# kpmrozowski/wut-cuda-orb-slam3

Hardware: NVIDIA B200
Metric: orb_extract_frames_per_s_752x480_1000kp (higher is better)
Workload: dtype u8

## Files before the change

### wut_cuda_orb_slam3_b200/csrc/api.cu

```cuda
#include <algorithm>
#include <atomic>
#include <climits>
#include <cfloat>
#include <cmath>
#include <cstdarg>
#include <cstdio>
#include <cstdlib>
#include <cstring>
#include <mutex>
#include <string>
#include <unordered_map>
#include <vector>

#include "orbx_internal.cuh"
#include "introsort_replay.h"
#include "synth.h"

namespace orbx {

static thread_local std::string t_err;
static std::atomic<long long> g_launches{0};

void count_launch(int n) { g_launches.fetch_add(n, std::memory_order_relaxed); }

int fail(int code, const char* fmt, ...)
{
    char buf[512];
    va_list ap;
    va_start(ap, fmt);
    vsnprintf(buf, sizeof buf, fmt, ap);
    va_end(ap);
    t_err = buf;
    return code;
}

#define CU(call)                                                                                         \
// ... 566 lines not shown
{
    if (!ex->profiling) return ORBX_OK;
    if (ex->ev_used == ex->ev_pool.size()) {
        cudaEvent_t e;
        CU(cudaEventCreate(&e));
        ex->ev_pool.push_back(e);
    }
    CU(cudaEventRecord(ex->ev_pool[ex->ev_used++], st));
    return ORBX_OK;
}

static int run_chunk(orbx_extractor* ex, Slot& s, const uint8_t* d_images, size_t frame_stride, size_t pitch, int frames,
                     int lap0, int lap1, orbx_keypoint* d_kps, uint8_t* d_desc, int capacity, int* d_n, int* d_nm,
                     cudaStream_t st)
{
    const FrameGeom& fg = ex->fg;
    int rc;
    ex->mirror_valid = false;
    if ((rc = prof_mark(ex, st))) return rc;
    CU(launch_pyramid(fg, s.ws, d_images, frame_stride, pitch, frames, st));
    if ((rc = prof_mark(ex, st))) return rc;
    static const char* fork_env = getenv("ORBX_BATCH_FORK");
    const bool fork = (fork_env ? atoi(fork_env) != 0 : true) && !ex->profiling && frames >= 8;
    if (fork) {
        if (!ex->side[0]) CU(cudaStreamCreateWithFlags(&ex->side[0], cudaStreamNonBlocking));
        if (!ex->ev_lvl[0]) CU(cudaEventCreateWithFlags(&ex->ev_lvl[0], cudaEventDisableTiming));
        if (!ex->ev_side[0]) CU(cudaEventCreateWithFlags(&ex->ev_side[0], cudaEventDisableTiming));
        CU(cudaEventRecord(ex->ev_lvl[0], st));
        CU(cudaStreamWaitEvent(ex->side[0], ex->ev_lvl[0], 0));
        CU(launch_fast(fg, s.ws, frames, st));
        CU(launch_blur(fg, s.ws, frames, ex->side[0]));
        CU(cudaEventRecord(ex->ev_side[0], ex->side[0]));
        CU(launch_octree(fg, s.ws, frames, st));
        CU(cudaStreamWaitEvent(st, ex->ev_side[0], 0));
    } else {
        CU(launch_fast(fg, s.ws, frames, st));
        if ((rc = prof_mark(ex, st))) return rc;
        CU(launch_blur(fg, s.ws, frames, st));
        if ((rc = prof_mark(ex, st))) return rc;
        CU(launch_octree(fg, s.ws, frames, st));
    }
    if ((rc = prof_mark(ex, st))) return rc;
    bool fused = false;
    CU(launch_orient_describe(fg, s.ws, frames, st, lap0, lap1, d_kps, d_desc, capacity, d_n, d_nm, &fused));
    if ((rc = prof_mark(ex, st))) return rc;
    if (!fused) CU(launch_pack(fg, s.ws, frames, lap0, lap1, d_kps, d_desc, capacity, d_n, d_nm, st));
    if ((rc = prof_mark(ex, st))) return rc;
    return ORBX_OK;
}

static int run_single_forked(orbx_extractor* ex, Slot& s, const uint8_t* d_image, size_t pitch, int lap0, int lap1,
                             orbx_keypoint* d_kps, uint8_t* d_desc, int capacity, int* d_n, int* d_nm, cudaStream_t st)
{
    const FrameGeom& fg = ex->fg;
    for (int l = 0; l < fg.nlevels; ++l) {
        if (!ex->side[l]) CU(cudaStreamCreateWithFlags(&ex->side[l], cudaStreamNonBlocking));
        if (!ex->ev_lvl[l]) CU(cudaEventCreateWithFlags(&ex->ev_lvl[l], cudaEventDisableTiming));
        if (!ex->ev_side[l]) CU(cudaEventCreateWithFlags(&ex->ev_side[l], cudaEventDisableTiming));
    }
    for (int l = 0; l < fg.nlevels; ++l) {
        CU(launch_pyramid(fg, s.ws, d_image, pitch * fg.rows, pitch, 1, st, l, l + 1));
        CU(cudaEventRecord(ex->ev_lvl[l], st));
        if (ex->mirror) {
            const LevelGeom& g = fg.L[l];
            const size_t bw = (size_t)g.w + 2 * kEdge;
            CU(cudaStreamWaitEvent(ex->mirror_stream, ex->ev_lvl[l], 0));
            CU(cudaMemcpy2DAsync(ex->h_mirror + ex->mirror_off[l], bw, s.ws.pyr + g.pyr_off + (kXPad - kEdge), g.pitch, bw, (size_t)g.rows_alloc,
// ... 1040 lines not shown
```

### wut_cuda_orb_slam3_b200/csrc/kernels_describe.cu

```cuda
#include <float.h>

#include <algorithm>
#include <cstdlib>
#include <mutex>

#include "orbx_internal.cuh"

namespace orbx {

namespace {

__constant__ int c_umax[16] = {15, 15, 15, 15, 14, 14, 14, 13, 13, 12, 11, 10, 9, 8, 6, 3};

__device__ float4 d_pattern_f[8][32];
__device__ uint4 d_mom_mask[16][2];

constexpr int BT_W = 128, BT_H = 32;
constexpr int BIN_P = 160;
constexpr int BIN_R = BT_H + 6;

__device__ __forceinline__ float fast_atan2_dev(float y, float x)
{
    const float scale = (float)(180.0 / 3.14159265358979323846);
    const float p1 = 0.9997878412794807f * scale, p3 = -0.3258083974640975f * scale;
    const float p5 = 0.1555786518463281f * scale, p7 = -0.04432655554792128f * scale;
    const float ax = fabsf(x), ay = fabsf(y);
    float a, c, c2;
    if (ax >= ay) {
        c = __fdiv_rn(ay, __fadd_rn(ax, (float)DBL_EPSILON));
        c2 = __fmul_rn(c, c);
        a = __fmul_rn(__fadd_rn(__fmul_rn(__fadd_rn(__fmul_rn(__fadd_rn(__fmul_rn(p7, c2), p5), c2), p3), c2), p1), c);
    } else {
        c = __fdiv_rn(ax, __fadd_rn(ay, (float)DBL_EPSILON));
        c2 = __fmul_rn(c, c);
        a = __fsub_rn(90.f, __fmul_rn(__fadd_rn(__fmul_rn(__fadd_rn(__fmul_rn(__fadd_rn(__fmul_rn(p7, c2), p5), c2), p3), c2), p1), c));
    }
    if (x < 0) a = __fsub_rn(180.f, a);
    if (y < 0) a = __fsub_rn(360.f, a);
    return a;
}

}

__global__ void __launch_bounds__(256) blur_kernel(const __grid_constant__ FrameGeom fg, Workspace ws)
{
    __shared__ __align__(128) uint8_t in[BIN_R * BIN_P];
    __shared__ __align__(16) uint32_t hb[BIN_R * BT_W];
    __shared__ __align__(16) uint8_t outt[BT_H * BT_W];
    const int tid = threadIdx.x;
    const int frame = blockIdx.y;
    int t = blockIdx.x, level = 0, tx_n = 0;
#pragma unroll 1
    for (int l = 0; l < fg.nlevels; ++l) {
        tx_n = (fg.L[l].w + BT_W - 1) / BT_W;
        const int nt = tx_n * ((fg.L[l].h + BT_H - 1) / BT_H);
        if (t < nt) { level = l; break; }
        t -= nt;
    }
    const LevelGeom& g = fg.L[level];
    const int tyi = t / tx_n;
    const int ty0 = tyi * BT_H, tx0 = (t - tyi * tx_n) * BT_W;
    const uint8_t* base = ws.pyr + g.pyr_off + (size_t)frame * g.pyr_frame_stride;
    const int brow0 = ty0 - 3 + kEdge, bcol0 = tx0 - 16 + kXPad;
// ... 200 lines not shown
            for (int r = 0; r < rows; r += 7) {
#pragma unroll
                for (int kk = 0; kk < 7; ++kk) {
                    if (r + kk < rows) {
                        hrow(r + kk + 6, W[(kk + 6) % 7]);
                        uint32_t o = 0;
#pragma unroll
                        for (int j = 0; j < 4; ++j) {
                            const uint32_t sum = 18u * (W[kk % 7][j] + W[(kk + 6) % 7][j]) + 34u * (W[(kk + 1) % 7][j] + W[(kk + 5) % 7][j]) +
                                                 48u * (W[(kk + 2) % 7][j] + W[(kk + 4) % 7][j]) + 56u * W[(kk + 3) % 7][j];
                            o |= ((sum + 32768u) >> 16) << (8 * j);
                        }
                        *reinterpret_cast<uint32_t*>(out) = o;
                        out += bpitch;
                    }
                }
            }
        }
        __syncwarp();
        if (lane == 0 && item + kBpStages * nw < total_items) issue(item + kBpStages * nw, sgi);
    }
}

struct FusedPack {
    int mode;
    orbx_keypoint* kps; uint8_t* desc; int capacity; int* n_out; int* n_mono;
};

constexpr int kOdStage = kDescBoxW * kDescBoxH;
#ifndef ORBX_OD_MINB
#define ORBX_OD_MINB 5
#endif

template <bool STAGED>
__global__ void __launch_bounds__(256, STAGED ? ORBX_OD_MINB : 1) orient_describe_kernel(const __grid_constant__ FrameGeom fg, Workspace ws, FusedPack fp)
{
    extern __shared__ __align__(128) uint8_t od_smem[];
    __shared__ __align__(8) uint64_t od_bar[8];
    const int lane = threadIdx.x & 31;
    const int slot = blockIdx.x * 8 + (threadIdx.x >> 5);
    const int frame = blockIdx.y;
    if (slot >= fg.kp_slots) return;
    static_assert((kMaxLevels & (kMaxLevels - 1)) == 0, "binary search over a power of two");
    int level = 0;
#pragma unroll
    for (int step = kMaxLevels / 2; step >= 1; step >>= 1)
        if (slot >= fg.L[level + step].kp_base) level += step;
    const LevelGeom& g = fg.L[level];
    const int i = slot - g.kp_base;
    int n_level, t_out = 0, nkp = 0;
    if (fp.mode) {
        const int c = lane < fg.nlevels ? ws.lvl_n[(size_t)frame * fg.nlevels + lane] : 0;
        int incl = c;
#pragma unroll
        for (int d = 1; d < 32; d <<= 1) {
            const int t = __shfl_up_sync(0xffffffffu, incl, d);
            if (lane >= d) incl += t;
        }
        n_level = __shfl_sync(0xffffffffu, c, level);
        t_out = __shfl_sync(0xffffffffu, incl - c, level) + i;
        nkp = __shfl_sync(0xffffffffu, incl, 31);
        if (slot == 0 && lane == 0) {
            fp.n_out[frame] = nkp;
            fp.n_mono[frame] = nkp > fp.capacity ? -1 : (fp.mode == 1 ? nkp : 0);
        }
    } else {
        n_level = ws.lvl_n[(size_t)frame * fg.nlevels + level];
    }
    if (i >= n_level) return;
    const uint32_t key = ws.lvl_kp[(size_t)frame * fg.kp_slots + slot];
    const int x = (int)(key & 0xfff) + kWinBorder, y = (int)((key >> 12) & 0xfff) + kWinBorder;

    constexpr bool staged = STAGED;
    const int warp = threadIdx.x >> 5;
    const int x0 = (x - 19) & ~15;
    const uint32_t stage_s = (uint32_t)__cvta_generic_to_shared(od_smem) + (uint32_t)warp * kOdStage;
    if (staged) {
        if (lane == 0) {
            mbar_init(&od_bar[warp], 1);
            mbar_expect_tx(&od_bar[warp], kDescBoxW * kDescBoxH);
            tma_load_3d(od_smem + warp * kOdStage, ws.tmap_desc + level, &od_bar[warp], x0, y - 20, frame);
        }
        __syncwarp();
    }

    int m10 = 0, m01 = 0;
    {
        const int v = lane - kHalfPatch;
        if (lane < 31) {
            const uint8_t* rowp = level_interior((const uint8_t*)ws.pyr, g, frame) + (ptrdiff_t)(y + v) * g.pitch + (x - kHalfPatch);
            const int mis16 = (int)((uintptr_t)rowp & 15);
            const int mis = mis16 & 3;
            const uint4* rq = reinterpret_cast<const uint4*>(rowp - mis16);
            const uint4 q0 = __ldg(rq), q1 = __ldg(rq + 1), q2 = __ldg(rq + 2);
            uint32_t w[12] = {q0.x, q0.y, q0.z, q0.w, q1.x, q1.y, q1.z, q1.w, q2.x, q2.y, q2.z, q2.w};
            if (mis16 & 4) {
#pragma unroll
                for (int j = 0; j < 11; ++j) w[j] = w[j + 1];
            }
            if (mis16 & 8) {
#pragma unroll
                for (int j = 0; j < 10; ++j) w[j] = w[j + 2];
            }
            const int av = v < 0 ? -v : v;
            const uint4 ma = d_mom_mask[av][0], mb = d_mom_mask[av][1];
            const uint32_t mk[8] = {ma.x, ma.y, ma.z, ma.w, mb.x, mb.y, mb.z, mb.w};
            const int sh = 8 * mis;
            int sum = 0;
#pragma unroll
            for (int j = 0; j < 8; ++j) {
                const uint32_t px = __funnelshift_r(w[j], w[j + 1], sh) & mk[j];
                const int u0 = -kHalfPatch + 4 * j;
                const uint32_t wt = (uint32_t)(u0 & 0xff) | ((uint32_t)((u0 + 1) & 0xff) << 8) | ((uint32_t)((u0 + 2) & 0xff) << 16) |
                                    ((uint32_t)((u0 + 3) & 0xff) << 24);
                asm("dp4a.u32.s32 %0, %1, %2, %0;" : "+r"(m10) : "r"(px), "r"(wt));
                sum = (int)__dp4a(px, 0x01010101u, (uint32_t)sum);
            }
            m01 = v * sum;
        }
#pragma unroll
        for (int d = 16; d >= 1; d >>= 1) {
            m10 += __shfl_xor_sync(0xffffffffu, m10, d);
            m01 += __shfl_xor_sync(0xffffffffu, m01, d);
        }
    }
    const float angle = fast_atan2_dev((float)m01, (float)m10);

    const float factorPI = (float)(3.14159265358979323846 / 180.f);
    const float arad = __fmul_rn(angle, factorPI);
    double sd, cd;
    sincos((double)arad, &sd, &cd);
    const float a = (float)cd, b = (float)sd;
    const uint8_t* center = ws.blur + g.blur_off + (size_t)frame * g.blur_frame_stride + (size_t)y * g.bpitch + x;
    const int step = g.bpitch;
    const float kMagic = 12582912.0f;
    const int kMagicBits = 0x4B400000;
    uint32_t val = 0;
    if (staged) {
        mbar_wait(&od_bar[warp], 0);
        const uint32_t cb = stage_s + 20 * kDescBoxW + (uint32_t)(x - x0);
#pragma unroll
        for (int k = 0; k < 8; ++k) {
            const float4 q = d_pattern_f[k][lane];
            const int iy0 = __float_as_int(__fadd_rn(__fadd_rn(__fmul_rn(q.x, b), __fmul_rn(q.y, a)), kMagic)) - kMagicBits;
            const int ix0 = __float_as_int(__fadd_rn(__fsub_rn(__fmul_rn(q.x, a), __fmul_rn(q.y, b)), kMagic)) - kMagicBits;
            const int iy1 = __float_as_int(__fadd_rn(__fadd_rn(__fmul_rn(q.z, b), __fmul_rn(q.w, a)), kMagic)) - kMagicBits;
            const int ix1 = __float_as_int(__fadd_rn(__fsub_rn(__fmul_rn(q.z, a), __fmul_rn(q.w, b)), kMagic)) - kMagicBits;
            uint32_t t0, t1;
            asm volatile("ld.shared.u8 %0, [%1];" : "=r"(t0) : "r"(cb + (uint32_t)(iy0 * kDescBoxW + ix0)));
            asm volatile("ld.shared.u8 %0, [%1];" : "=r"(t1) : "r"(cb + (uint32_t)(iy1 * kDescBoxW + ix1)));
            val |= (uint32_t)(t0 < t1) << k;
        }
    } else
#pragma unroll
    for (int k = 0; k < 8; ++k) {
        const float4 q = d_pattern_f[k][lane];
        const int iy0 = __float_as_int(__fadd_rn(__fadd_rn(__fmul_rn(q.x, b), __fmul_rn(q.y, a)), kMagic)) - kMagicBits;
        const int ix0 = __float_as_int(__fadd_rn(__fsub_rn(__fmul_rn(q.x, a), __fmul_rn(q.y, b)), kMagic)) - kMagicBits;
        const int iy1 = __float_as_int(__fadd_rn(__fadd_rn(__fmul_rn(q.z, b), __fmul_rn(q.w, a)), kMagic)) - kMagicBits;
        const int ix1 = __float_as_int(__fadd_rn(__fsub_rn(__fmul_rn(q.z, a), __fmul_rn(q.w, b)), kMagic)) - kMagicBits;
        const int t0 = __ldg(center + iy0 * step + ix0), t1 = __ldg(center + iy1 * step + ix1);
        val |= (uint32_t)(t0 < t1) << k;
    }
    ws.lvl_desc[((size_t)frame * fg.kp_slots + slot) * 32 + lane] = (uint8_t)val;
    if (lane == 0) ws.lvl_angle[(size_t)frame * fg.kp_slots + slot] = angle;
    if (fp.mode && nkp <= fp.capacity) {
        const int dst = fp.mode == 1 ? t_out : nkp - 1 - t_out;
        fp.desc[((size_t)frame * fp.capacity + dst) * 32 + lane] = (uint8_t)val;
        if (lane < 7) {
            float px = (float)x, py = (float)y;
            if (level != 0) { px = __fmul_rn(px, g.scale); py = __fmul_rn(py, g.scale); }
            uint32_t w;
            switch (lane) {
                case 0: w = __float_as_uint(px); break;
                case 1: w = __float_as_uint(py); break;
                case 2: w = __float_as_uint(g.kp_size); break;
                case 3: w = __float_as_uint(angle); break;
                case 4: w = __float_as_uint((float)(key >> 24)); break;
                case 5: w = (uint32_t)level; break;
                default: w = 0xffffffffu; break;
            }
            reinterpret_cast<uint32_t*>(fp.kps + (size_t)frame * fp.capacity + dst)[lane] = w;
        }
    }
}

template <int T>
__global__ void __launch_bounds__(T) pack_kernel(const __grid_constant__ FrameGeom fg, Workspace ws, int lap0, int lap1,
                                                 orbx_keypoint* __restrict__ kps, uint8_t* __restrict__ desc, int capacity,
                                                 int* __restrict__ n_out, int* __restrict__ n_mono)
{
    __shared__ int lvl_off[kMaxLevels + 1];
    __shared__ int warp_cnt[T / 32];
    __shared__ int carry;
    const int tid = threadIdx.x, lane = tid & 31, warp = tid >> 5;
    const int frame = blockIdx.x;
    if (warp == 0) {
        static_assert(kMaxLevels <= 32, "one lane per level");
        const int c = lane < fg.nlevels ? ws.lvl_n[(size_t)frame * fg.nlevels + lane] : 0;
        int incl = c;
#pragma unroll
        for (int d = 1; d < 32; d <<= 1) {
            const int t = __shfl_up_sync(0xffffffffu, incl, d);
            if (lane >= d) incl += t;
        }
        if (lane < fg.nlevels) lvl_off[lane] = incl - c;
        if (lane == fg.nlevels - 1) lvl_off[fg.nlevels] = incl;
// ... 99 lines not shown
    };
    static const int umax[16] = {15, 15, 15, 15, 14, 14, 14, 13, 13, 12, 11, 10, 9, 8, 6, 3};
    float4 pf[8][32];
    for (int lane = 0; lane < 32; ++lane)
        for (int k = 0; k < 8; ++k) {
            const int8_t* t = pat + 4 * (8 * lane + k);
            pf[k][lane] = make_float4((float)t[0], (float)t[1], (float)t[2], (float)t[3]);
        }
    uint32_t mask[16][8];
    for (int av = 0; av < 16; ++av)
        for (int j = 0; j < 8; ++j) {
            uint32_t m = 0;
            for (int bb = 0; bb < 4; ++bb) {
                const int u = -15 + 4 * j + bb;
                if ((u < 0 ? -u : u) <= umax[av]) m |= 0xffu << (8 * bb);
            }
            mask[av][j] = m;
        }
    cudaError_t e = cudaMemcpyToSymbol(d_pattern_f, pf, sizeof pf);
    if (e != cudaSuccess) return e;
    return cudaMemcpyToSymbol(d_mom_mask, mask, sizeof mask);
}

cudaError_t launch_orient_describe(const FrameGeom& fg, const Workspace& ws, int n_frames, cudaStream_t st, int lap0, int lap1,
                                   orbx_keypoint* d_kps, uint8_t* d_desc, int capacity, int* d_n_out, int* d_n_mono, bool* fused)
{
    FusedPack fp{};
    static const bool no_fuse = getenv("ORBX_NO_FUSED_PACK") != nullptr;
    if (d_kps && d_desc && d_n_out && d_n_mono && !no_fuse && fg.kp_slots > 0 && n_frames < 8) {
        if (lap1 < kEdge || lap0 >= fg.cols || lap0 > lap1) fp.mode = 1;
        else if (lap0 <= kEdge && lap1 >= fg.cols) fp.mode = 2;
        fp.kps = d_kps; fp.desc = d_desc; fp.capacity = capacity; fp.n_out = d_n_out; fp.n_mono = d_n_mono;
    }
    if (fused) *fused = fp.mode != 0;
    static bool filled[64] = {false};
    static std::mutex mu;
    int dev = 0;
    cudaGetDevice(&dev);
    std::lock_guard<std::mutex> lock(mu);
    if (!filled[dev & 63]) {
        cudaError_t e = fill_describe_tables();
        if (e != cudaSuccess) return e;
        filled[dev & 63] = true;
    }
    dim3 grid((fg.kp_slots + 7) / 8, n_frames);
    static const char* od_env = getenv("ORBX_DESC_STAGED");
    if (ws.tmap_desc && (od_env ? atoi(od_env) != 0 : true)) orient_describe_kernel<true><<<grid, 256, 8 * kOdStage, st>>>(fg, ws, fp);
    else orient_describe_kernel<false><<<grid, 256, 0, st>>>(fg, ws, fp);
    count_launch();
    return cudaGetLastError();
}

cudaError_t launch_pack(const FrameGeom& fg, const Workspace& ws, int n_frames, int lap0, int lap1, orbx_keypoint* d_kps,
                        uint8_t* d_desc, int capacity, int* d_n_out, int* d_n_mono, cudaStream_t st)
{
    if (n_frames >= 8) pack_kernel<256><<<n_frames, 256, 0, st>>>(fg, ws, lap0, lap1, d_kps, d_desc, capacity, d_n_out, d_n_mono);
    else pack_kernel<1024><<<n_frames, 1024, 0, st>>>(fg, ws, lap0, lap1, d_kps, d_desc, capacity, d_n_out, d_n_mono);
    count_launch();
    return cudaGetLastError();
}

}
```

### wut_cuda_orb_slam3_b200/csrc/kernels_octree.cu

```cuda
#include <stdlib.h>

#include <mutex>

#include "introsort_replay.h"
#include "orbx_internal.cuh"

namespace orbx {

namespace {

constexpr int kSortBitsMax = 12;

struct Smem {
    int* bstart;
    int* cursor;
    int* warp_tmp;
    int* sort_stk;
    uint32_t* nbeg[2];
    uint32_t* ncnt[2];
    uint32_t* nx[2];
    uint32_t* ndep[2];
    uint32_t* npre[2];
    uint32_t* cc;
    int* sa;
    int* sb;
    int* sc;
// ... 199 lines not shown
__host__ __device__ inline int octree_sort_depth(int depth, int root_bits)
{
    const int d = (kSortBitsMax - root_bits) / 2;
    return d < depth ? (d > 0 ? d : 0) : depth;
}

int octree_bins(const LevelGeom& g) { return 1 << (g.root_bits + 2 * octree_sort_depth(g.depth, g.root_bits)); }

size_t octree_smem_bytes(int M, int NB)
{
    size_t b = 0;
    b += sizeof(uint32_t) * (size_t)M * 10;
    b += sizeof(uint32_t) * (size_t)M * 4;
    b += sizeof(int) * (size_t)M * 5;
    b += 8;
    b += sizeof(unsigned long long) * (size_t)M * 2;
    const size_t cur = sizeof(int) * (size_t)NB;
    return sizeof(int) * (64 + 224) + sizeof(int) * ((size_t)NB + 2) + (b > cur ? b : cur);
}

#ifndef ORBX_OCT_THREADS_PER_SM
#define ORBX_OCT_THREADS_PER_SM 1024
#endif
template <int T>
__global__ void __launch_bounds__(T, ORBX_OCT_THREADS_PER_SM / T) octree_kernel(const __grid_constant__ FrameGeom fg, Workspace ws, int M, int NB,
                                                   int level_base, int* __restrict__ err_flag)
{
    extern __shared__ __align__(16) unsigned char smem_raw[];
    __shared__ int s_nL, s_nS, s_total;

    const int tid = threadIdx.x, lane = tid & 31, warp = tid >> 5;
    const int frame = blockIdx.x, level = level_base + blockIdx.y;
    const LevelGeom& g = fg.L[level];
    const int N = g.nfeat;
    long long* dbg = (ws.dbg && frame == 0 && level == ws.dbg_level && tid == 0) ? ws.dbg : nullptr;
    long long t_prev = dbg ? clock64() : 0;
#define OCT_MARK(slot) do { if (dbg) { const long long t_now = clock64(); dbg[slot] += t_now - t_prev; t_prev = t_now; } } while (0)
    long long t_fine = t_prev;
#define OCT_FINE(slot) do { if (dbg) { const long long t_now = clock64(); dbg[slot] += t_now - t_fine; t_fine = t_now; } } while (0)
    const int winW = g.w - 2 * kWinBorder, winH = g.h - 2 * kWinBorder;

    Smem S;
    {
        unsigned char* p = smem_raw;
        S.warp_tmp = (int*)p; p += sizeof(int) * 64;
        S.sort_stk = (int*)p; p += sizeof(int) * 224;
        S.bstart = (int*)p; p += sizeof(int) * ((size_t)NB + 2);
        S.cursor = (int*)p;
        for (int b = 0; b < 2; ++b) {
            S.nbeg[b] = (uint32_t*)p; p += 4 * (size_t)M;
            S.ncnt[b] = (uint32_t*)p; p += 4 * (size_t)M;
// ... 313 lines not shown
            const int i = i0 + u;
            if (i < nL) {
                const uint32_t beg = S.nbeg[a][i], cnt = S.ncnt[a][i];
                for (uint32_t j = lane; j < cnt; j += 32) {
                    const uint32_t pl = K[beg + j], kk = K2[beg + j];
                    const unsigned long long v = ((unsigned long long)((pl & 0xff000000u) | (0xffffffu - (pl & 0xffffffu))) << 32) | kk;
                    best[u] = v > best[u] ? v : best[u];
                }
            }
        }
#pragma unroll
        for (int u = 0; u < RU; ++u) {
#pragma unroll
            for (int d = 16; d >= 1; d >>= 1) {
                const unsigned long long o = __shfl_xor_sync(0xffffffffu, best[u], d);
                best[u] = o > best[u] ? o : best[u];
            }
            if (lane == 0 && i0 + u < nL) out_kp[i0 + u] = (uint32_t)best[u];
        }
    }
    if (tid == 0) *out_n = nL;
    OCT_MARK(6);
    if (dbg) dbg[9] = n;
#undef OCT_MARK
#undef OCT_FINE
}

cudaError_t octree_prepare()
{
    cudaError_t e = cudaFuncSetAttribute(octree_kernel<256>, cudaFuncAttributeMaxDynamicSharedMemorySize, 200 * 1024);
    if (e != cudaSuccess) return e;
    e = cudaFuncSetAttribute(octree_kernel<64>, cudaFuncAttributeMaxDynamicSharedMemorySize, 200 * 1024);
    if (e != cudaSuccess) return e;
    e = cudaFuncSetAttribute(octree_kernel<128>, cudaFuncAttributeMaxDynamicSharedMemorySize, 200 * 1024);
    if (e != cudaSuccess) return e;
    e = cudaFuncSetAttribute(octree_kernel<512>, cudaFuncAttributeMaxDynamicSharedMemorySize, 200 * 1024);
    if (e != cudaSuccess) return e;
    return cudaFuncSetAttribute(octree_kernel<1024>, cudaFuncAttributeMaxDynamicSharedMemorySize, 200 * 1024);
}

size_t octree_smem_for(const FrameGeom& fg, int level_lo, int level_hi)
{
    int M = 1, NB = 1;
    for (int l = level_lo; l < level_hi; ++l) {
        M = M > fg.L[l].kp_cap ? M : fg.L[l].kp_cap;
        const int nb = octree_bins(fg.L[l]);
        NB = NB > nb ? NB : nb;
    }
    return octree_smem_bytes(M, NB);
}

static int* g_err_flag[64] = {nullptr};

int octree_take_error_flag()
{
    int dev = 0;
    cudaGetDevice(&dev);
    int* p = g_err_flag[dev & 63];
    if (!p) return 0;
    int v = 0;
    if (cudaMemcpy(&v, p, sizeof(int), cudaMemcpyDeviceToHost) != cudaSuccess) return 0;
    if (v) cudaMemset(p, 0, sizeof(int));
    return v;
}

cudaError_t launch_octree(const FrameGeom& fg, const Workspace& ws, int n_frames, cudaStream_t st, int level_lo, int level_hi)
{
    if (level_hi <= 0) level_hi = fg.nlevels;
    if (level_lo >= level_hi) return cudaSuccess;
    int M = 1, NB = 1;
    for (int l = level_lo; l < level_hi; ++l) {
        M = M > fg.L[l].kp_cap ? M : fg.L[l].kp_cap;
        const int nb = octree_bins(fg.L[l]);
        NB = NB > nb ? NB : nb;
    }
    static const int t_override = getenv("ORBX_OCTREE_THREADS") ? atoi(getenv("ORBX_OCTREE_THREADS")) : 0;
    int T = n_frames >= 8 ? 256 : 1024;
    if (t_override == 64 || t_override == 128 || t_override == 256 || t_override == 512 || t_override == 1024) T = t_override;
    const size_t smem = octree_smem_bytes(M, NB);
    if (smem > 200 * 1024) return cudaErrorInvalidConfiguration;
    int dev = 0;
    cudaGetDevice(&dev);
    if (!g_err_flag[dev & 63]) {
        static std::mutex mu;
        std::lock_guard<std::mutex> lock(mu);
        if (!g_err_flag[dev & 63]) {
            int* p = nullptr;
            cudaError_t e = cudaMalloc(&p, sizeof(int));
            if (e != cudaSuccess) return e;
            cudaMemset(p, 0, sizeof(int));
            g_err_flag[dev & 63] = p;
        }
    }
    dim3 grid(n_frames, level_hi - level_lo);
    if (T == 64) octree_kernel<64><<<grid, 64, smem, st>>>(fg, ws, M, NB, level_lo, g_err_flag[dev & 63]);
    else if (T == 128) octree_kernel<128><<<grid, 128, smem, st>>>(fg, ws, M, NB, level_lo, g_err_flag[dev & 63]);
    else if (T == 1024) octree_kernel<1024><<<grid, 1024, smem, st>>>(fg, ws, M, NB, level_lo, g_err_flag[dev & 63]);
    else if (T == 512) octree_kernel<512><<<grid, 512, smem, st>>>(fg, ws, M, NB, level_lo, g_err_flag[dev & 63]);
    else octree_kernel<256><<<grid, 256, smem, st>>>(fg, ws, M, NB, level_lo, g_err_flag[dev & 63]);
    count_launch();
    return cudaGetLastError();
}

}
```

### wut_cuda_orb_slam3_b200/csrc/orbx_internal.cuh

```cuda
#pragma once
#include <cuda.h>
#include <cuda_runtime.h>
#include <stdint.h>

#include "../../include/orbx.h"

namespace orbx {

constexpr int kEdge = ORBX_EDGE_THRESHOLD;
constexpr int kXPad = 32;
constexpr int kWinBorder = 16;
constexpr int kMaxLevels = ORBX_MAX_LEVELS;
constexpr int kMaxCellDim = 70;
constexpr int kMaxDim = 4128;
constexpr int kHalfPatch = 15;
constexpr int kDescBoxW = 80, kDescBoxH = 40;

struct LevelGeom {
    int w, h;
    int pitch;
    int rows_alloc;
    unsigned long long pyr_off;
    unsigned long long pyr_frame_stride;
    int bpitch;
// ... 78 lines not shown
    const uint32_t a = (uint32_t)__cvta_generic_to_shared(bar);
    uint32_t ok;
    do {
        asm volatile("{\n\t.reg .pred p;\n\tmbarrier.try_wait.parity.shared::cta.b64 p, [%1], %2;\n\tselp.u32 %0, 1, 0, p;\n\t}"
                     : "=r"(ok) : "r"(a), "r"(parity) : "memory");
    } while (!ok);
}
__device__ __forceinline__ void tma_load_3d(void* smem_dst, const CUtensorMap* map, uint64_t* bar, int x, int y, int z)
{
    asm volatile("cp.async.bulk.tensor.3d.shared::cluster.global.mbarrier::complete_tx::bytes [%0], [%1, {%2, %3, %4}], [%5];"
                 ::"r"((uint32_t)__cvta_generic_to_shared(smem_dst)), "l"(map), "r"(x), "r"(y), "r"(z),
                 "r"((uint32_t)__cvta_generic_to_shared(bar)) : "memory");
}
#endif

void count_launch(int n = 1);

cudaError_t launch_pyramid(const FrameGeom& fg, const Workspace& ws, const uint8_t* d_images, size_t frame_stride,
                           size_t pitch, int n_frames, cudaStream_t st, int level_lo = 0, int level_hi = 0);
cudaError_t launch_cvt_gray(const uint8_t* d_src, size_t src_pitch, size_t src_frame_stride, int channels, int rgb, int n_frames,
                            int rows, int cols, uint8_t* d_dst, size_t dst_pitch, size_t dst_frame_stride, cudaStream_t st);
cudaError_t launch_fast(const FrameGeom& fg, const Workspace& ws, int n_frames, cudaStream_t st, int level_lo = 0, int level_hi = 0);
cudaError_t launch_blur(const FrameGeom& fg, const Workspace& ws, int n_frames, cudaStream_t st);
cudaError_t launch_octree(const FrameGeom& fg, const Workspace& ws, int n_frames, cudaStream_t st, int level_lo = 0, int level_hi = 0);
cudaError_t launch_orient_describe(const FrameGeom& fg, const Workspace& ws, int n_frames, cudaStream_t st, int lap0 = 0, int lap1 = 0,
                                   orbx_keypoint* d_kps = nullptr, uint8_t* d_desc = nullptr, int capacity = 0, int* d_n_out = nullptr,
                                   int* d_n_mono = nullptr, bool* fused = nullptr);
cudaError_t launch_pack(const FrameGeom& fg, const Workspace& ws, int n_frames, int lap0, int lap1,
                        orbx_keypoint* d_kps, uint8_t* d_desc, int capacity, int* d_n_out, int* d_n_mono,
                        cudaStream_t st);
size_t octree_smem_for(const FrameGeom& fg, int level_lo, int level_hi);
int octree_take_error_flag();
cudaError_t octree_prepare();

cudaError_t launch_knn2(const uint8_t* d_q, int nq, const uint8_t* d_db, long long ndb, int index_base, int32_t* d_idx,
                        int32_t* d_dist, cudaStream_t st, void* workspace = nullptr);
size_t knn2_workspace_bytes(int nq, long long ndb);
cudaError_t launch_knn2_merge(const int32_t* d_idx_sh, const int32_t* d_dist_sh, int n_shards, int nq, int32_t* d_idx,
                              int32_t* d_dist, cudaStream_t st, size_t shard_stride = 0);
cudaError_t launch_popc_bench(unsigned long long* d_sink, int iters, int blocks, cudaStream_t st);

struct StereoArgs {
    const uint8_t* pyrL; const uint8_t* pyrR;
    unsigned long long offR[kMaxLevels];
    int frameL, frameR;
    const orbx_keypoint* kpL; const uint8_t* descL; int nL;
    const orbx_keypoint* kpR; const uint8_t* descR; int nR;
// ... 126 lines not shown
```

Baseline: 165,800.

## Fuse orientation and descriptor computation into the octree kernel for batched frames

For batched runs (eight or more frames) where the per-level keypoint budget is small, the octree kernel now computes orientation and the rBRIEF descriptor for its surviving keypoints. It reuses its shared memory as per-warp TMA staging buffers, so the separate orient_describe launch is skipped. The shared descriptor body moves into a header and its lookup tables are passed as device pointers. In exchange, the blur stream must now finish before the octree starts, so the blur/octree overlap is lost. Describe work also runs inside one block per level and frame, which may cut parallelism compared with the standalone kernel.

```diff
diff --git a/wut_cuda_orb_slam3_b200/csrc/api.cu b/wut_cuda_orb_slam3_b200/csrc/api.cu
--- a/wut_cuda_orb_slam3_b200/csrc/api.cu
+++ b/wut_cuda_orb_slam3_b200/csrc/api.cu
@@ -12,6 +12,7 @@
 #include <unordered_map>
 #include <vector>
 
+#include "describe_body.cuh"
 #include "orbx_internal.cuh"
 #include "introsort_replay.h"
 #include "synth.h"
@@ -624,6 +625,14 @@
     if ((rc = prof_mark(ex, st))) return rc;
     static const char* fork_env = getenv("ORBX_BATCH_FORK");
     const bool fork = (fork_env ? atoi(fork_env) != 0 : true) && !ex->profiling && frames >= 8;
+    constexpr int kOdFusedMaxKeys = 336;
+    static const char* od_fused_env = getenv("ORBX_OCT_DESC_FUSED");
+    int max_keys = 0;
+    for (int l = 0; l < fg.nlevels; ++l) max_keys = std::max(max_keys, fg.L[l].nfeat);
+    const bool od_fused = (od_fused_env ? atoi(od_fused_env) != 0 : max_keys <= kOdFusedMaxKeys) && frames >= 8 && describe_staged(s.ws);
+    DescTables tables{};
+    if (od_fused) CU(describe_tables(&tables));
+    const DescTables* desc = od_fused ? &tables : nullptr;
     if (fork) {
         if (!ex->side[0]) CU(cudaStreamCreateWithFlags(&ex->side[0], cudaStreamNonBlocking));
         if (!ex->ev_lvl[0]) CU(cudaEventCreateWithFlags(&ex->ev_lvl[0], cudaEventDisableTiming));
@@ -633,18 +642,23 @@
         CU(launch_fast(fg, s.ws, frames, st));
         CU(launch_blur(fg, s.ws, frames, ex->side[0]));
         CU(cudaEventRecord(ex->ev_side[0], ex->side[0]));
-        CU(launch_octree(fg, s.ws, frames, st));
-        CU(cudaStreamWaitEvent(st, ex->ev_side[0], 0));
+        if (od_fused) {
+            CU(cudaStreamWaitEvent(st, ex->ev_side[0], 0));
+            CU(launch_octree(fg, s.ws, frames, st, 0, 0, desc));
+        } else {
+            CU(launch_octree(fg, s.ws, frames, st));
+            CU(cudaStreamWaitEvent(st, ex->ev_side[0], 0));
+        }
     } else {
         CU(launch_fast(fg, s.ws, frames, st));
         if ((rc = prof_mark(ex, st))) return rc;
         CU(launch_blur(fg, s.ws, frames, st));
         if ((rc = prof_mark(ex, st))) return rc;
-        CU(launch_octree(fg, s.ws, frames, st));
+        CU(launch_octree(fg, s.ws, frames, st, 0, 0, desc));
     }
     if ((rc = prof_mark(ex, st))) return rc;
     bool fused = false;
-    CU(launch_orient_describe(fg, s.ws, frames, st, lap0, lap1, d_kps, d_desc, capacity, d_n, d_nm, &fused));
+    if (!od_fused) CU(launch_orient_describe(fg, s.ws, frames, st, lap0, lap1, d_kps, d_desc, capacity, d_n, d_nm, &fused));
     if ((rc = prof_mark(ex, st))) return rc;
     if (!fused) CU(launch_pack(fg, s.ws, frames, lap0, lap1, d_kps, d_desc, capacity, d_n, d_nm, st));
     if ((rc = prof_mark(ex, st))) return rc;
diff --git a/wut_cuda_orb_slam3_b200/csrc/describe_body.cuh b/wut_cuda_orb_slam3_b200/csrc/describe_body.cuh
--- /dev/null
+++ b/wut_cuda_orb_slam3_b200/csrc/describe_body.cuh
@@ -0,0 +1,161 @@
+#pragma once
+#include <float.h>
+
+#include "orbx_internal.cuh"
+
+namespace orbx {
+
+struct DescTables {
+    const float4* pattern;
+    const uint4* mom_mask;
+};
+
+struct FusedPack {
+    int mode;
+    orbx_keypoint* kps; uint8_t* desc; int capacity; int* n_out; int* n_mono;
+};
+
+constexpr int kOdStage = kDescBoxW * kDescBoxH;
+
+__device__ __forceinline__ float fast_atan2_dev(float y, float x)
+{
+    const float scale = (float)(180.0 / 3.14159265358979323846);
+    const float p1 = 0.9997878412794807f * scale, p3 = -0.3258083974640975f * scale;
+    const float p5 = 0.1555786518463281f * scale, p7 = -0.04432655554792128f * scale;
+    const float ax = fabsf(x), ay = fabsf(y);
+    float a, c, c2;
+    if (ax >= ay) {
+        c = __fdiv_rn(ay, __fadd_rn(ax, (float)DBL_EPSILON));
+        c2 = __fmul_rn(c, c);
+        a = __fmul_rn(__fadd_rn(__fmul_rn(__fadd_rn(__fmul_rn(__fadd_rn(__fmul_rn(p7, c2), p5), c2), p3), c2), p1), c);
+    } else {
+        c = __fdiv_rn(ax, __fadd_rn(ay, (float)DBL_EPSILON));
+        c2 = __fmul_rn(c, c);
+        a = __fsub_rn(90.f, __fmul_rn(__fadd_rn(__fmul_rn(__fadd_rn(__fmul_rn(__fadd_rn(__fmul_rn(p7, c2), p5), c2), p3), c2), p1), c));
+    }
+    if (x < 0) a = __fsub_rn(180.f, a);
+    if (y < 0) a = __fsub_rn(360.f, a);
+    return a;
+}
+
+template <bool STAGED>
+__device__ __forceinline__ void describe_key(const FrameGeom& fg, const Workspace& ws, int frame, int level, int slot, uint32_t key,
+                                             uint8_t* stage, uint64_t* bar, uint32_t parity, const FusedPack& fp, int t_out, int nkp,
+                                             const DescTables& tb)
+{
+    const int lane = threadIdx.x & 31;
+    const LevelGeom& g = fg.L[level];
+    const int x = (int)(key & 0xfff) + kWinBorder, y = (int)((key >> 12) & 0xfff) + kWinBorder;
+
+    const int x0 = (x - 19) & ~15;
+    const uint32_t stage_s = (uint32_t)__cvta_generic_to_shared(stage);
+    if (STAGED) {
+        if (lane == 0) {
+            mbar_expect_tx(bar, kDescBoxW * kDescBoxH);
+            tma_load_3d(stage, ws.tmap_desc + level, bar, x0, y - 20, frame);
+        }
+        __syncwarp();
+    }
+
+    int m10 = 0, m01 = 0;
+    {
+        const int v = lane - kHalfPatch;
+        if (lane < 31) {
+            const uint8_t* rowp = level_interior((const uint8_t*)ws.pyr, g, frame) + (ptrdiff_t)(y + v) * g.pitch + (x - kHalfPatch);
+            const int mis16 = (int)((uintptr_t)rowp & 15);
+            const int mis = mis16 & 3;
+            const uint4* rq = reinterpret_cast<const uint4*>(rowp - mis16);
+            const uint4 q0 = __ldg(rq), q1 = __ldg(rq + 1), q2 = __ldg(rq + 2);
+            uint32_t w[12] = {q0.x, q0.y, q0.z, q0.w, q1.x, q1.y, q1.z, q1.w, q2.x, q2.y, q2.z, q2.w};
+            if (mis16 & 4) {
+#pragma unroll
+                for (int j = 0; j < 11; ++j) w[j] = w[j + 1];
+            }
+            if (mis16 & 8) {
+#pragma unroll
+                for (int j = 0; j < 10; ++j) w[j] = w[j + 2];
+            }
+            const int av = v < 0 ? -v : v;
+            const uint4 ma = tb.mom_mask[2 * av], mb = tb.mom_mask[2 * av + 1];
+            const uint32_t mk[8] = {ma.x, ma.y, ma.z, ma.w, mb.x, mb.y, mb.z, mb.w};
+            const int sh = 8 * mis;
+            int sum = 0;
+#pragma unroll
+            for (int j = 0; j < 8; ++j) {
+                const uint32_t px = __funnelshift_r(w[j], w[j + 1], sh) & mk[j];
+                const int u0 = -kHalfPatch + 4 * j;
+                const uint32_t wt = (uint32_t)(u0 & 0xff) | ((uint32_t)((u0 + 1) & 0xff) << 8) | ((uint32_t)((u0 + 2) & 0xff) << 16) |
+                                    ((uint32_t)((u0 + 3) & 0xff) << 24);
+                asm("dp4a.u32.s32 %0, %1, %2, %0;" : "+r"(m10) : "r"(px), "r"(wt));
+                sum = (int)__dp4a(px, 0x01010101u, (uint32_t)sum);
+            }
+            m01 = v * sum;
+        }
+#pragma unroll
+        for (int d = 16; d >= 1; d >>= 1) {
+            m10 += __shfl_xor_sync(0xffffffffu, m10, d);
+            m01 += __shfl_xor_sync(0xffffffffu, m01, d);
+        }
+    }
+    const float angle = fast_atan2_dev((float)m01, (float)m10);
+
+    const float factorPI = (float)(3.14159265358979323846 / 180.f);
+    const float arad = __fmul_rn(angle, factorPI);
+    double sd, cd;
+    sincos((double)arad, &sd, &cd);
+    const float a = (float)cd, b = (float)sd;
+    const uint8_t* center = ws.blur + g.blur_off + (size_t)frame * g.blur_frame_stride + (size_t)y * g.bpitch + x;
+    const int step = g.bpitch;
+    const float kMagic = 12582912.0f;
+    const int kMagicBits = 0x4B400000;
+    uint32_t val = 0;
+    if (STAGED) {
+        mbar_wait(bar, parity);
+        const uint32_t cb = stage_s + 20 * kDescBoxW + (uint32_t)(x - x0);
+#pragma unroll
+        for (int k = 0; k < 8; ++k) {
+            const float4 q = tb.pattern[k * 32 + lane];
+            const int iy0 = __float_as_int(__fadd_rn(__fadd_rn(__fmul_rn(q.x, b), __fmul_rn(q.y, a)), kMagic)) - kMagicBits;
+            const int ix0 = __float_as_int(__fadd_rn(__fsub_rn(__fmul_rn(q.x, a), __fmul_rn(q.y, b)), kMagic)) - kMagicBits;
+            const int iy1 = __float_as_int(__fadd_rn(__fadd_rn(__fmul_rn(q.z, b), __fmul_rn(q.w, a)), kMagic)) - kMagicBits;
+            const int ix1 = __float_as_int(__fadd_rn(__fsub_rn(__fmul_rn(q.z, a), __fmul_rn(q.w, b)), kMagic)) - kMagicBits;
+            uint32_t t0, t1;
+            asm volatile("ld.shared.u8 %0, [%1];" : "=r"(t0) : "r"(cb + (uint32_t)(iy0 * kDescBoxW + ix0)));
+            asm volatile("ld.shared.u8 %0, [%1];" : "=r"(t1) : "r"(cb + (uint32_t)(iy1 * kDescBoxW + ix1)));
+            val |= (uint32_t)(t0 < t1) << k;
+        }
+    } else
+#pragma unroll
+    for (int k = 0; k < 8; ++k) {
+        const float4 q = tb.pattern[k * 32 + lane];
+        const int iy0 = __float_as_int(__fadd_rn(__fadd_rn(__fmul_rn(q.x, b), __fmul_rn(q.y, a)), kMagic)) - kMagicBits;
+        const int ix0 = __float_as_int(__fadd_rn(__fsub_rn(__fmul_rn(q.x, a), __fmul_rn(q.y, b)), kMagic)) - kMagicBits;
+        const int iy1 = __float_as_int(__fadd_rn(__fadd_rn(__fmul_rn(q.z, b), __fmul_rn(q.w, a)), kMagic)) - kMagicBits;
+        const int ix1 = __float_as_int(__fadd_rn(__fsub_rn(__fmul_rn(q.z, a), __fmul_rn(q.w, b)), kMagic)) - kMagicBits;
+        const int t0 = __ldg(center + iy0 * step + ix0), t1 = __ldg(center + iy1 * step + ix1);
+        val |= (uint32_t)(t0 < t1) << k;
+    }
+    ws.lvl_desc[((size_t)frame * fg.kp_slots + slot) * 32 + lane] = (uint8_t)val;
+    if (lane == 0) ws.lvl_angle[(size_t)frame * fg.kp_slots + slot] = angle;
+    if (fp.mode && nkp <= fp.capacity) {
+        const int dst = fp.mode == 1 ? t_out : nkp - 1 - t_out;
+        fp.desc[((size_t)frame * fp.capacity + dst) * 32 + lane] = (uint8_t)val;
+        if (lane < 7) {
+            float px = (float)x, py = (float)y;
+            if (level != 0) { px = __fmul_rn(px, g.scale); py = __fmul_rn(py, g.scale); }
+            uint32_t w;
+            switch (lane) {
+                case 0: w = __float_as_uint(px); break;
+                case 1: w = __float_as_uint(py); break;
+                case 2: w = __float_as_uint(g.kp_size); break;
+                case 3: w = __float_as_uint(angle); break;
+                case 4: w = __float_as_uint((float)(key >> 24)); break;
+                case 5: w = (uint32_t)level; break;
+                default: w = 0xffffffffu; break;
+            }
+            reinterpret_cast<uint32_t*>(fp.kps + (size_t)frame * fp.capacity + dst)[lane] = w;
+        }
+    }
+}
+
+}
diff --git a/wut_cuda_orb_slam3_b200/csrc/kernels_describe.cu b/wut_cuda_orb_slam3_b200/csrc/kernels_describe.cu
--- a/wut_cuda_orb_slam3_b200/csrc/kernels_describe.cu
+++ b/wut_cuda_orb_slam3_b200/csrc/kernels_describe.cu
@@ -1,9 +1,9 @@
-#include <float.h>
 
 #include <algorithm>
 #include <cstdlib>
 #include <mutex>
 
+#include "describe_body.cuh"
 #include "orbx_internal.cuh"
 
 namespace orbx {
@@ -18,27 +18,6 @@
 constexpr int BT_W = 128, BT_H = 32;
 constexpr int BIN_P = 160;
 constexpr int BIN_R = BT_H + 6;
-
-__device__ __forceinline__ float fast_atan2_dev(float y, float x)
-{
-    const float scale = (float)(180.0 / 3.14159265358979323846);
-    const float p1 = 0.9997878412794807f * scale, p3 = -0.3258083974640975f * scale;
-    const float p5 = 0.1555786518463281f * scale, p7 = -0.04432655554792128f * scale;
-    const float ax = fabsf(x), ay = fabsf(y);
-    float a, c, c2;
-    if (ax >= ay) {
-        c = __fdiv_rn(ay, __fadd_rn(ax, (float)DBL_EPSILON));
-        c2 = __fmul_rn(c, c);
-        a = __fmul_rn(__fadd_rn(__fmul_rn(__fadd_rn(__fmul_rn(__fadd_rn(__fmul_rn(p7, c2), p5), c2), p3), c2), p1), c);
-    } else {
-        c = __fdiv_rn(ax, __fadd_rn(ay, (float)DBL_EPSILON));
-        c2 = __fmul_rn(c, c);
-        a = __fsub_rn(90.f, __fmul_rn(__fadd_rn(__fmul_rn(__fadd_rn(__fmul_rn(__fadd_rn(__fmul_rn(p7, c2), p5), c2), p3), c2), p1), c));
-    }
-    if (x < 0) a = __fsub_rn(180.f, a);
-    if (y < 0) a = __fsub_rn(360.f, a);
-    return a;
-}
 
 }
 
@@ -285,12 +264,6 @@
     }
 }
 
-struct FusedPack {
-    int mode;
-    orbx_keypoint* kps; uint8_t* desc; int capacity; int* n_out; int* n_mono;
-};
-
-constexpr int kOdStage = kDescBoxW * kDescBoxH;
 #ifndef ORBX_OD_MINB
 #define ORBX_OD_MINB 5
 #endif
@@ -332,120 +305,10 @@
     }
     if (i >= n_level) return;
     const uint32_t key = ws.lvl_kp[(size_t)frame * fg.kp_slots + slot];
-    const int x = (int)(key & 0xfff) + kWinBorder, y = (int)((key >> 12) & 0xfff) + kWinBorder;
-
-    constexpr bool staged = STAGED;
     const int warp = threadIdx.x >> 5;
-    const int x0 = (x - 19) & ~15;
-    const uint32_t stage_s = (uint32_t)__cvta_generic_to_shared(od_smem) + (uint32_t)warp * kOdStage;
-    if (staged) {
-        if (lane == 0) {
-            mbar_init(&od_bar[warp], 1);
-            mbar_expect_tx(&od_bar[warp], kDescBoxW * kDescBoxH);
-            tma_load_3d(od_smem + warp * kOdStage, ws.tmap_desc + level, &od_bar[warp], x0, y - 20, frame);
-        }
-        __syncwarp();
-    }
-
-    int m10 = 0, m01 = 0;
-    {
-        const int v = lane - kHalfPatch;
-        if (lane < 31) {
-            const uint8_t* rowp = level_interior((const uint8_t*)ws.pyr, g, frame) + (ptrdiff_t)(y + v) * g.pitch + (x - kHalfPatch);
-            const int mis16 = (int)((uintptr_t)rowp & 15);
-            const int mis = mis16 & 3;
-            const uint4* rq = reinterpret_cast<const uint4*>(rowp - mis16);
-            const uint4 q0 = __ldg(rq), q1 = __ldg(rq + 1), q2 = __ldg(rq + 2);
-            uint32_t w[12] = {q0.x, q0.y, q0.z, q0.w, q1.x, q1.y, q1.z, q1.w, q2.x, q2.y, q2.z, q2.w};
-            if (mis16 & 4) {
-#pragma unroll
-                for (int j = 0; j < 11; ++j) w[j] = w[j + 1];
-            }
-            if (mis16 & 8) {
-#pragma unroll
-                for (int j = 0; j < 10; ++j) w[j] = w[j + 2];
-            }
-            const int av = v < 0 ? -v : v;
-            const uint4 ma = d_mom_mask[av][0], mb = d_mom_mask[av][1];
-            const uint32_t mk[8] = {ma.x, ma.y, ma.z, ma.w, mb.x, mb.y, mb.z, mb.w};
-            const int sh = 8 * mis;
-            int sum = 0;
-#pragma unroll
-            for (int j = 0; j < 8; ++j) {
-                const uint32_t px = __funnelshift_r(w[j], w[j + 1], sh) & mk[j];
-                const int u0 = -kHalfPatch + 4 * j;
-                const uint32_t wt = (uint32_t)(u0 & 0xff) | ((uint32_t)((u0 + 1) & 0xff) << 8) | ((uint32_t)((u0 + 2) & 0xff) << 16) |
-                                    ((uint32_t)((u0 + 3) & 0xff) << 24);
-                asm("dp4a.u32.s32 %0, %1, %2, %0;" : "+r"(m10) : "r"(px), "r"(wt));
-                sum = (int)__dp4a(px, 0x01010101u, (uint32_t)sum);
-            }
-            m01 = v * sum;
-        }
-#pragma unroll
-        for (int d = 16; d >= 1; d >>= 1) {
-            m10 += __shfl_xor_sync(0xffffffffu, m10, d);
-            m01 += __shfl_xor_sync(0xffffffffu, m01, d);
-        }
-    }
-    const float angle = fast_atan2_dev((float)m01, (float)m10);
-
-    const float factorPI = (float)(3.14159265358979323846 / 180.f);
-    const float arad = __fmul_rn(angle, factorPI);
-    double sd, cd;
-    sincos((double)arad, &sd, &cd);
-    const float a = (float)cd, b = (float)sd;
-    const uint8_t* center = ws.blur + g.blur_off + (size_t)frame * g.blur_frame_stride + (size_t)y * g.bpitch + x;
-    const int step = g.bpitch;
-    const float kMagic = 12582912.0f;
-    const int kMagicBits = 0x4B400000;
-    uint32_t val = 0;
-    if (staged) {
-        mbar_wait(&od_bar[warp], 0);
-        const uint32_t cb = stage_s + 20 * kDescBoxW + (uint32_t)(x - x0);
-#pragma unroll
-        for (int k = 0; k < 8; ++k) {
-            const float4 q = d_pattern_f[k][lane];
-            const int iy0 = __float_as_int(__fadd_rn(__fadd_rn(__fmul_rn(q.x, b), __fmul_rn(q.y, a)), kMagic)) - kMagicBits;
-            const int ix0 = __float_as_int(__fadd_rn(__fsub_rn(__fmul_rn(q.x, a), __fmul_rn(q.y, b)), kMagic)) - kMagicBits;
-            const int iy1 = __float_as_int(__fadd_rn(__fadd_rn(__fmul_rn(q.z, b), __fmul_rn(q.w, a)), kMagic)) - kMagicBits;
-            const int ix1 = __float_as_int(__fadd_rn(__fsub_rn(__fmul_rn(q.z, a), __fmul_rn(q.w, b)), kMagic)) - kMagicBits;
-            uint32_t t0, t1;
-            asm volatile("ld.shared.u8 %0, [%1];" : "=r"(t0) : "r"(cb + (uint32_t)(iy0 * kDescBoxW + ix0)));
-            asm volatile("ld.shared.u8 %0, [%1];" : "=r"(t1) : "r"(cb + (uint32_t)(iy1 * kDescBoxW + ix1)));
-            val |= (uint32_t)(t0 < t1) << k;
-        }
-    } else
-#pragma unroll
-    for (int k = 0; k < 8; ++k) {
-        const float4 q = d_pattern_f[k][lane];
-        const int iy0 = __float_as_int(__fadd_rn(__fadd_rn(__fmul_rn(q.x, b), __fmul_rn(q.y, a)), kMagic)) - kMagicBits;
-        const int ix0 = __float_as_int(__fadd_rn(__fsub_rn(__fmul_rn(q.x, a), __fmul_rn(q.y, b)), kMagic)) - kMagicBits;
-        const int iy1 = __float_as_int(__fadd_rn(__fadd_rn(__fmul_rn(q.z, b), __fmul_rn(q.w, a)), kMagic)) - kMagicBits;
-        const int ix1 = __float_as_int(__fadd_rn(__fsub_rn(__fmul_rn(q.z, a), __fmul_rn(q.w, b)), kMagic)) - kMagicBits;
-        const int t0 = __ldg(center + iy0 * step + ix0), t1 = __ldg(center + iy1 * step + ix1);
-        val |= (uint32_t)(t0 < t1) << k;
-    }
-    ws.lvl_desc[((size_t)frame * fg.kp_slots + slot) * 32 + lane] = (uint8_t)val;
-    if (lane == 0) ws.lvl_angle[(size_t)frame * fg.kp_slots + slot] = angle;
-    if (fp.mode && nkp <= fp.capacity) {
-        const int dst = fp.mode == 1 ? t_out : nkp - 1 - t_out;
-        fp.desc[((size_t)frame * fp.capacity + dst) * 32 + lane] = (uint8_t)val;
-        if (lane < 7) {
-            float px = (float)x, py = (float)y;
-            if (level != 0) { px = __fmul_rn(px, g.scale); py = __fmul_rn(py, g.scale); }
-            uint32_t w;
-            switch (lane) {
-                case 0: w = __float_as_uint(px); break;
-                case 1: w = __float_as_uint(py); break;
-                case 2: w = __float_as_uint(g.kp_size); break;
-                case 3: w = __float_as_uint(angle); break;
-                case 4: w = __float_as_uint((float)(key >> 24)); break;
-                case 5: w = (uint32_t)level; break;
-                default: w = 0xffffffffu; break;
-            }
-            reinterpret_cast<uint32_t*>(fp.kps + (size_t)frame * fp.capacity + dst)[lane] = w;
-        }
-    }
+    if (STAGED && lane == 0) mbar_init(&od_bar[warp], 1);
+    describe_key<STAGED>(fg, ws, frame, level, slot, key, od_smem + warp * kOdStage, &od_bar[warp], 0, fp, t_out, nkp,
+                         DescTables{&d_pattern_f[0][0], &d_mom_mask[0][0]});
 }
 
 template <int T>
@@ -591,18 +454,10 @@
     return cudaMemcpyToSymbol(d_mom_mask, mask, sizeof mask);
 }
 
-cudaError_t launch_orient_describe(const FrameGeom& fg, const Workspace& ws, int n_frames, cudaStream_t st, int lap0, int lap1,
-                                   orbx_keypoint* d_kps, uint8_t* d_desc, int capacity, int* d_n_out, int* d_n_mono, bool* fused)
-{
-    FusedPack fp{};
-    static const bool no_fuse = getenv("ORBX_NO_FUSED_PACK") != nullptr;
-    if (d_kps && d_desc && d_n_out && d_n_mono && !no_fuse && fg.kp_slots > 0 && n_frames < 8) {
-        if (lap1 < kEdge || lap0 >= fg.cols || lap0 > lap1) fp.mode = 1;
-        else if (lap0 <= kEdge && lap1 >= fg.cols) fp.mode = 2;
-        fp.kps = d_kps; fp.desc = d_desc; fp.capacity = capacity; fp.n_out = d_n_out; fp.n_mono = d_n_mono;
-    }
-    if (fused) *fused = fp.mode != 0;
+cudaError_t describe_tables(DescTables* tb)
+{
     static bool filled[64] = {false};
+    static DescTables addr[64];
     static std::mutex mu;
     int dev = 0;
     cudaGetDevice(&dev);
@@ -610,11 +465,39 @@
     if (!filled[dev & 63]) {
         cudaError_t e = fill_describe_tables();
         if (e != cudaSuccess) return e;
+        void* p = nullptr;
+        if ((e = cudaGetSymbolAddress(&p, d_pattern_f)) != cudaSuccess) return e;
+        addr[dev & 63].pattern = (const float4*)p;
+        if ((e = cudaGetSymbolAddress(&p, d_mom_mask)) != cudaSuccess) return e;
+        addr[dev & 63].mom_mask = (const uint4*)p;
         filled[dev & 63] = true;
     }
+    *tb = addr[dev & 63];
+    return cudaSuccess;
+}
+
+bool describe_staged(const Workspace& ws)
+{
+    static const char* od_env = getenv("ORBX_DESC_STAGED");
+    return ws.tmap_desc && (od_env ? atoi(od_env) != 0 : true);
+}
+
+cudaError_t launch_orient_describe(const FrameGeom& fg, const Workspace& ws, int n_frames, cudaStream_t st, int lap0, int lap1,
+                                   orbx_keypoint* d_kps, uint8_t* d_desc, int capacity, int* d_n_out, int* d_n_mono, bool* fused)
+{
+    FusedPack fp{};
+    static const bool no_fuse = getenv("ORBX_NO_FUSED_PACK") != nullptr;
+    if (d_kps && d_desc && d_n_out && d_n_mono && !no_fuse && fg.kp_slots > 0 && n_frames < 8) {
+        if (lap1 < kEdge || lap0 >= fg.cols || lap0 > lap1) fp.mode = 1;
+        else if (lap0 <= kEdge && lap1 >= fg.cols) fp.mode = 2;
+        fp.kps = d_kps; fp.desc = d_desc; fp.capacity = capacity; fp.n_out = d_n_out; fp.n_mono = d_n_mono;
+    }
+    if (fused) *fused = fp.mode != 0;
+    DescTables tb;
+    cudaError_t e = describe_tables(&tb);
+    if (e != cudaSuccess) return e;
     dim3 grid((fg.kp_slots + 7) / 8, n_frames);
-    static const char* od_env = getenv("ORBX_DESC_STAGED");
-    if (ws.tmap_desc && (od_env ? atoi(od_env) != 0 : true)) orient_describe_kernel<true><<<grid, 256, 8 * kOdStage, st>>>(fg, ws, fp);
+    if (describe_staged(ws)) orient_describe_kernel<true><<<grid, 256, 8 * kOdStage, st>>>(fg, ws, fp);
     else orient_describe_kernel<false><<<grid, 256, 0, st>>>(fg, ws, fp);
     count_launch();
     return cudaGetLastError();
diff --git a/wut_cuda_orb_slam3_b200/csrc/kernels_octree.cu b/wut_cuda_orb_slam3_b200/csrc/kernels_octree.cu
--- a/wut_cuda_orb_slam3_b200/csrc/kernels_octree.cu
+++ b/wut_cuda_orb_slam3_b200/csrc/kernels_octree.cu
@@ -1,7 +1,10 @@
 #include <stdlib.h>
 
+#include <algorithm>
+
 #include <mutex>
 
+#include "describe_body.cuh"
 #include "introsort_replay.h"
 #include "orbx_internal.cuh"
 
@@ -247,11 +250,18 @@
 #ifndef ORBX_OCT_THREADS_PER_SM
 #define ORBX_OCT_THREADS_PER_SM 1024
 #endif
-template <int T>
-__global__ void __launch_bounds__(T, ORBX_OCT_THREADS_PER_SM / T) octree_kernel(const __grid_constant__ FrameGeom fg, Workspace ws, int M, int NB,
-                                                   int level_base, int* __restrict__ err_flag)
-{
-    extern __shared__ __align__(16) unsigned char smem_raw[];
+#ifndef ORBX_OCT_DESC_THREADS_PER_SM
+#define ORBX_OCT_DESC_THREADS_PER_SM 1024
+#endif
+#ifndef ORBX_OCT_DESC_T
+#define ORBX_OCT_DESC_T 256
+#endif
+constexpr int kOdT = ORBX_OCT_DESC_T;
+template <int T, bool DESC = false>
+__global__ void __launch_bounds__(T, (DESC ? ORBX_OCT_DESC_THREADS_PER_SM : ORBX_OCT_THREADS_PER_SM) / T) octree_kernel(const __grid_constant__ FrameGeom fg, Workspace ws, int M, int NB,
+                                                   int level_base, int* __restrict__ err_flag, DescTables tb)
+{
+    extern __shared__ __align__(128) unsigned char smem_raw[];
     __shared__ int s_nL, s_nS, s_total;
 
     const int tid = threadIdx.x, lane = tid & 31, warp = tid >> 5;
@@ -611,6 +621,25 @@
     if (tid == 0) *out_n = nL;
     OCT_MARK(6);
     if (dbg) dbg[9] = n;
+
+    if constexpr (DESC) {
+        __shared__ __align__(8) uint64_t od_bar[T / 32];
+        asm volatile("fence.proxy.async.shared::cta;" ::: "memory");
+        __syncthreads();
+        uint8_t* stage = smem_raw + (size_t)warp * kOdStage;
+        if (lane == 0) mbar_init(&od_bar[warp], 1);
+        __syncwarp();
+        const FusedPack no_pack{};
+        uint32_t parity = 0;
+        for (int i = warp; i < nL; i += T / 32) {
+            const int slot = g.kp_base + i;
+            const uint32_t key = ws.lvl_kp[(size_t)frame * fg.kp_slots + slot];
+            if (lane == 0) asm volatile("fence.proxy.async.shared::cta;" ::: "memory");
+            describe_key<true>(fg, ws, frame, level, slot, key, stage, &od_bar[warp], parity, no_pack, 0, 0, tb);
+            parity ^= 1u;
+            __syncwarp();
+        }
+    }
 #undef OCT_MARK
 #undef OCT_FINE
 }
@@ -625,6 +654,8 @@
     if (e != cudaSuccess) return e;
     e = cudaFuncSetAttribute(octree_kernel<512>, cudaFuncAttributeMaxDynamicSharedMemorySize, 200 * 1024);
     if (e != cudaSuccess) return e;
+    e = cudaFuncSetAttribute(octree_kernel<kOdT, true>, cudaFuncAttributeMaxDynamicSharedMemorySize, 200 * 1024);
+    if (e != cudaSuccess) return e;
     return cudaFuncSetAttribute(octree_kernel<1024>, cudaFuncAttributeMaxDynamicSharedMemorySize, 200 * 1024);
 }
 
@@ -653,7 +684,8 @@
     return v;
 }
 
-cudaError_t launch_octree(const FrameGeom& fg, const Workspace& ws, int n_frames, cudaStream_t st, int level_lo, int level_hi)
+cudaError_t launch_octree(const FrameGeom& fg, const Workspace& ws, int n_frames, cudaStream_t st, int level_lo, int level_hi,
+                          const DescTables* desc)
 {
     if (level_hi <= 0) level_hi = fg.nlevels;
     if (level_lo >= level_hi) return cudaSuccess;
@@ -666,7 +698,8 @@
     static const int t_override = getenv("ORBX_OCTREE_THREADS") ? atoi(getenv("ORBX_OCTREE_THREADS")) : 0;
     int T = n_frames >= 8 ? 256 : 1024;
     if (t_override == 64 || t_override == 128 || t_override == 256 || t_override == 512 || t_override == 1024) T = t_override;
-    const size_t smem = octree_smem_bytes(M, NB);
+    size_t smem = octree_smem_bytes(M, NB);
+    if (desc) smem = std::max(smem, (size_t)(kOdT / 32) * kOdStage);
     if (smem > 200 * 1024) return cudaErrorInvalidConfiguration;
     int dev = 0;
     cudaGetDevice(&dev);
@@ -682,11 +715,13 @@
         }
     }
     dim3 grid(n_frames, level_hi - level_lo);
-    if (T == 64) octree_kernel<64><<<grid, 64, smem, st>>>(fg, ws, M, NB, level_lo, g_err_flag[dev & 63]);
-    else if (T == 128) octree_kernel<128><<<grid, 128, smem, st>>>(fg, ws, M, NB, level_lo, g_err_flag[dev & 63]);
-    else if (T == 1024) octree_kernel<1024><<<grid, 1024, smem, st>>>(fg, ws, M, NB, level_lo, g_err_flag[dev & 63]);
-    else if (T == 512) octree_kernel<512><<<grid, 512, smem, st>>>(fg, ws, M, NB, level_lo, g_err_flag[dev & 63]);
-    else octree_kernel<256><<<grid, 256, smem, st>>>(fg, ws, M, NB, level_lo, g_err_flag[dev & 63]);
+    const DescTables tb = desc ? *desc : DescTables{};
+    if (desc) octree_kernel<kOdT, true><<<grid, kOdT, smem, st>>>(fg, ws, M, NB, level_lo, g_err_flag[dev & 63], tb);
+    else if (T == 64) octree_kernel<64><<<grid, 64, smem, st>>>(fg, ws, M, NB, level_lo, g_err_flag[dev & 63], tb);
+    else if (T == 128) octree_kernel<128><<<grid, 128, smem, st>>>(fg, ws, M, NB, level_lo, g_err_flag[dev & 63], tb);
+    else if (T == 1024) octree_kernel<1024><<<grid, 1024, smem, st>>>(fg, ws, M, NB, level_lo, g_err_flag[dev & 63], tb);
+    else if (T == 512) octree_kernel<512><<<grid, 512, smem, st>>>(fg, ws, M, NB, level_lo, g_err_flag[dev & 63], tb);
+    else octree_kernel<256><<<grid, 256, smem, st>>>(fg, ws, M, NB, level_lo, g_err_flag[dev & 63], tb);
     count_launch();
     return cudaGetLastError();
 }
diff --git a/wut_cuda_orb_slam3_b200/csrc/orbx_internal.cuh b/wut_cuda_orb_slam3_b200/csrc/orbx_internal.cuh
--- a/wut_cuda_orb_slam3_b200/csrc/orbx_internal.cuh
+++ b/wut_cuda_orb_slam3_b200/csrc/orbx_internal.cuh
@@ -124,7 +124,11 @@
                             int rows, int cols, uint8_t* d_dst, size_t dst_pitch, size_t dst_frame_stride, cudaStream_t st);
 cudaError_t launch_fast(const FrameGeom& fg, const Workspace& ws, int n_frames, cudaStream_t st, int level_lo = 0, int level_hi = 0);
 cudaError_t launch_blur(const FrameGeom& fg, const Workspace& ws, int n_frames, cudaStream_t st);
-cudaError_t launch_octree(const FrameGeom& fg, const Workspace& ws, int n_frames, cudaStream_t st, int level_lo = 0, int level_hi = 0);
+struct DescTables;
+cudaError_t describe_tables(DescTables* tb);
+bool describe_staged(const Workspace& ws);
+cudaError_t launch_octree(const FrameGeom& fg, const Workspace& ws, int n_frames, cudaStream_t st, int level_lo = 0, int level_hi = 0,
+                          const DescTables* desc = nullptr);
 cudaError_t launch_orient_describe(const FrameGeom& fg, const Workspace& ws, int n_frames, cudaStream_t st, int lap0 = 0, int lap1 = 0,
                                    orbx_keypoint* d_kps = nullptr, uint8_t* d_desc = nullptr, int capacity = 0, int* d_n_out = nullptr,
                                    int* d_n_mono = nullptr, bool* fused = nullptr);
```

Measured after the change: 168,800, median of 6. 1.02x the previous value.
